# tskare/gpuaudiobench

Measured on AMD Instinct MI355X. Metric: audio_buffers_per_sec, higher is better.
Workload: dtype f32

## Files before the change

gpuaudiobench_amd/csrc/k_conv_accel.hip:

```cpp
#include <hip/hip_runtime.h>
#include <hip/hip_ext.h>

#include <cmath>
#include <cstdlib>
#include <algorithm>
#include <chrono>
#include <memory>
#include <mutex>
#include <string>
#include <thread>
#include <type_traits>
#include <utility>
#include <vector>

#include "gab_common.hpp"
#include "gab_fft.hpp"
#include "gab_plan.hpp"
#include "k_conv_fdl.hpp"

namespace gab {
namespace fft {

void build_twiddles(float* t) {
    for (int m = 0; m < kTwiddleN; ++m) {
// ... 380 lines not shown
    const float* __restrict__ hist, const float4* __restrict__ pmF, cf* __restrict__ carry,
    const cf* __restrict__ tw, int head) {
    __shared__ cf lds[2 * kLdsHalf];
    const int tid = threadIdx.x;
    const int q = blockIdx.x;
    const cf* const hp = reinterpret_cast<const cf*>(hist) + (size_t)q * kSlots * kB;
    cf* const cp = carry + (size_t)q * kCarrySlots * kB;
    using FB = fft::BlockFFT<kNB, 16, false>;
    using FBi = fft::BlockFFT<kNB, 16, true>;
    cf* const X = lds;
    cf* const Y = lds + kLdsHalf;
    cf zb[16];
    typename FB::Bases twb_base;
    FB::load_twiddles(twb_base, tw, tid);
#pragma unroll
    for (int r = 0; r < 16; ++r)
        zb[r] = hp[((head + 1 + (r >> 1)) & (kSlots - 1)) * kB + (r & 1) * kThreads + tid];
    float4 cb[16];
    load_spectra<kNB, 16>(cb, pmF + (size_t)q * kBinsB, tid);
    typename FB::Twiddles twb;
    FB::expand_twiddles(twb_base, twb);
    FB::run(zb, X, Y, twb, tid);
    cf zpb[16];
    partner_exchange<kNB, 16, true>(zb, zpb, X, tid);
    spectral_product<kNB, 16>(zb, zpb, cb, tid);
    FBi::template run<typename FB::Twiddles, 4>(zb, Y, X, twb, tid);
    cf* const c1 = cp + ((head + 1) & (kCarrySlots - 1)) * kB;
    cf* const c2 = cp + ((head + 2) & (kCarrySlots - 1)) * kB;
    c1[tid] = zb[12];
    c1[tid + kThreads] = zb[13];
    c2[tid] = zb[14];
    c2[tid + kThreads] = zb[15];
}

constexpr unsigned kRtSentinel = 0xffa5c3e1u;
__device__ __forceinline__ bool rt_pending(unsigned w) { return (w >> 24) == (kRtSentinel >> 24); }
constexpr size_t kRtUploadPiece = (size_t(4) << 20) - 256;
constexpr int kRtPollLimit = 1 << 21;
constexpr int kRtMaxGroups = 40;
constexpr size_t kBatchChunk = 256;
struct ConvRoundTrip {
    unsigned* stage;
    float* park;
    float* h_out;
    unsigned* counters;
    unsigned* done;
    const unsigned* landed;
    unsigned* error;
    unsigned epoch;
    int groups;
    unsigned bound[kRtMaxGroups + 1];
};

#ifdef GAB_ABLATE
__device__ unsigned long long g_rt_stamps[65 * 4];
#define GAB_RT_STAMP_MIN(g, i) do { if (threadIdx.x == 0) atomicMin(&g_rt_stamps[(g) * 4 + (i)], (unsigned long long)__builtin_amdgcn_s_memrealtime()); } while (0)
#define GAB_RT_STAMP_MAX(g, i) do { if (threadIdx.x == 0) atomicMax(&g_rt_stamps[(g) * 4 + (i)], (unsigned long long)__builtin_amdgcn_s_memrealtime()); } while (0)
#else
#define GAB_RT_STAMP_MIN(g, i) do {} while (0)
#define GAB_RT_STAMP_MAX(g, i) do {} while (0)
#endif

__device__ __forceinline__ unsigned rt_peek(const unsigned* p) {
    return __hip_atomic_load(p, __ATOMIC_RELAXED, __HIP_MEMORY_SCOPE_SYSTEM);
}
constexpr unsigned kRtErrWait = 1u, kRtErrTorn = 2u;

__global__ __launch_bounds__(kThreads) void conv_round_trip_check_kernel(unsigned* __restrict__ stage, const float* __restrict__ hist,
                                                                        unsigned* __restrict__ verdict, int slot) {
    const int tid = threadIdx.x, q = blockIdx.x;
    const cf* const hp = reinterpret_cast<const cf*>(hist) + ((size_t)q * kSlots + slot) * kB;
    unsigned* const row = stage + (size_t)(2 * q) * kB;
    const cf c0 = hp[tid], c1 = hp[tid + kThreads];
    const unsigned v0 = rt_peek(row + tid), v1 = rt_peek(row + tid + kThreads), v2 = rt_peek(row + kB + tid), v3 = rt_peek(row + kB + tid + kThreads);
    const bool torn = v0 != __float_as_uint(c0.x) || v2 != __float_as_uint(c0.y) || v1 != __float_as_uint(c1.x) || v3 != __float_as_uint(c1.y);
    if (torn) __hip_atomic_fetch_or(verdict, kRtErrTorn, __ATOMIC_RELAXED, __HIP_MEMORY_SCOPE_SYSTEM);
    __hip_atomic_store(row + tid, kRtSentinel, __ATOMIC_RELAXED, __HIP_MEMORY_SCOPE_SYSTEM);
    __hip_atomic_store(row + tid + kThreads, kRtSentinel, __ATOMIC_RELAXED, __HIP_MEMORY_SCOPE_SYSTEM);
    __hip_atomic_store(row + kB + tid, kRtSentinel, __ATOMIC_RELAXED, __HIP_MEMORY_SCOPE_SYSTEM);
    __hip_atomic_store(row + kB + tid + kThreads, kRtSentinel, __ATOMIC_RELAXED, __HIP_MEMORY_SCOPE_SYSTEM);
}

__global__ __launch_bounds__(kThreads, 2) void conv_round_trip_kernel(
    ConvRoundTrip rt, float* __restrict__ hist, const float4* __restrict__ pmA, const float4* __restrict__ pmB,
    const cf* __restrict__ tw, int T, int head) {
    __shared__ cf lds[2 * kLdsHalf];
    __shared__ int s_word;
    cf* const lds0 = lds;
    cf* const lds1 = lds + kLdsHalf;
    const int tid = threadIdx.x;
    const int q = blockIdx.x;
    const int ta = 2 * q;
    int g = 0;
    while (q >= (int)rt.bound[g + 1]) ++g;
    GAB_RT_STAMP_MIN(g, 0);
    cf* const hp = reinterpret_cast<cf*>(hist) + (size_t)q * kSlots * kB;
    using FA = fft::BlockFFT<kNA, 4, false>;
    using FAi = fft::BlockFFT<kNA, 4, true>;
    using FB = fft::BlockFFT<kNB, 16, false>;
    using FBi = fft::BlockFFT<kNB, 16, true>;

    cf zb[16];
    typename FB::Bases twb_base;
    FB::load_twiddles(twb_base, tw, tid);
#pragma unroll
    for (int r = 0; r < 16; ++r) zb[r] = hp[((head + (r >> 1)) & (kSlots - 1)) * kB + (r & 1) * kThreads + tid];
    const cf prev0 = zb[14], prev1 = zb[15];
    {
        float4 cb[16];
        load_spectra<kNB, 16>(cb, pmB + (size_t)q * kBinsB, tid);
        __builtin_amdgcn_sched_barrier(0);
        typename FB::Twiddles twb;
        FB::expand_twiddles(twb_base, twb);
        FB::run(zb, lds1, lds0, twb, tid);
        cf zpb[16];
        partner_exchange<kNB, 16, true>(zb, zpb, lds1, tid);
        spectral_product<kNB, 16>(zb, zpb, cb, tid);
        FBi::template run<typename FB::Twiddles, 2>(zb, lds0, lds1, twb, tid);
    }
    const cf far0 = zb[14], far1 = zb[15];

    float4 ca[4];
    load_spectra<kNA, 4>(ca, pmA + (size_t)q * kBinsA, tid);
    typename FA::Twiddles twa;
    {
        typename FA::Bases twa_base;
        FA::load_twiddles(twa_base, tw, tid);
        FA::expand_twiddles(twa_base, twa);
    }

    const unsigned* const row = rt.stage + (size_t)ta * kB;
    if (tid == 0) {
        int tries = 0, bad = 0;
        while (rt_pending(rt_peek(row + 2 * kB - 1))) {
            if ((++tries & 63) == 0 && rt_peek(rt.landed) == rt.epoch) break;
            if (tries > kRtPollLimit) { bad = 1; break; }
            __builtin_amdgcn_s_sleep(30);
        }
        s_word = bad;
    }
    __syncthreads();
    bool gave_up = s_word != 0;
    unsigned w[4];
    {
        int tries = 0;
        for (;;) {
            w[0] = rt_peek(row + tid);
            w[1] = rt_peek(row + tid + kThreads);
            w[2] = rt_peek(row + kB + tid);
            w[3] = rt_peek(row + kB + tid + kThreads);
            if (gave_up || !(rt_pending(w[0]) || rt_pending(w[1]) || rt_pending(w[2]) || rt_pending(w[3]))) break;
            if ((++tries & 15) == 0 && __hip_atomic_load(rt.landed, __ATOMIC_ACQUIRE, __HIP_MEMORY_SCOPE_SYSTEM) == rt.epoch) {
                w[0] = rt_peek(row + tid);
                w[1] = rt_peek(row + tid + kThreads);
                w[2] = rt_peek(row + kB + tid);
                w[3] = rt_peek(row + kB + tid + kThreads);
                break;
            }
            if (tries > kRtPollLimit) { gave_up = true; break; }
            __builtin_amdgcn_s_sleep(10);
        }
    }
    GAB_RT_STAMP_MAX(g, 1);
    if (gave_up) __hip_atomic_store(rt.error, kRtErrWait, __ATOMIC_RELAXED, __HIP_MEMORY_SCOPE_SYSTEM);

    cf za[4];
    za[0] = prev0;
    za[1] = prev1;
    za[2] = mk(__uint_as_float(w[0]), __uint_as_float(w[2]));
    za[3] = mk(__uint_as_float(w[1]), __uint_as_float(w[3]));
    hp[head * kB + tid] = za[2];
    hp[head * kB + kThreads + tid] = za[3];
    __syncthreads();
    FA::run(za, lds0, lds1, twa, tid);
    {
        cf zpa[4];
        partner_exchange<kNA, 4, true>(za, zpa, lds0, tid);
        spectral_product<kNA, 4>(za, zpa, ca, tid);
    }
    FAi::run(za, lds1, lds0, twa, tid);
    float ya0 = 0.f, yb0 = 0.f, ya1 = 0.f, yb1 = 0.f;
    ya0 += za[2].x; yb0 += za[2].y; ya1 += za[3].x; yb1 += za[3].y;
    ya0 += far0.x; yb0 += far0.y; ya1 += far1.x; yb1 += far1.y;

    {
        unsigned long long* const p0 = reinterpret_cast<unsigned long long*>(rt.park + (size_t)T * tid + ta);
        unsigned long long* const p1 = reinterpret_cast<unsigned long long*>(rt.park + (size_t)T * (tid + kThreads) + ta);
        const unsigned long long v0 = ((unsigned long long)__float_as_uint(yb0) << 32) | __float_as_uint(ya0);
        const unsigned long long v1 = ((unsigned long long)__float_as_uint(yb1) << 32) | __float_as_uint(ya1);
        __hip_atomic_store(p0, v0, __ATOMIC_RELAXED, __HIP_MEMORY_SCOPE_AGENT);
        __hip_atomic_store(p1, v1, __ATOMIC_RELAXED, __HIP_MEMORY_SCOPE_AGENT);
    }
    asm volatile("s_waitcnt vmcnt(0)" ::: "memory");
    __syncthreads();
    GAB_RT_STAMP_MAX(g, 2);
    const int first = rt.bound[g];
    const int members = (int)rt.bound[g + 1] - first;
    unsigned* const gw = rt.counters + 32 * g;
    if (tid == 0) {
        const unsigned old = __hip_atomic_fetch_add(&gw[0], 1u, __ATOMIC_RELAXED, __HIP_MEMORY_SCOPE_AGENT);
        int role = 1;
        if (old + 1u == rt.epoch * (unsigned)members) {
            role = 2;
            __hip_atomic_store(&gw[1], 0u, __ATOMIC_RELAXED, __HIP_MEMORY_SCOPE_AGENT);
            asm volatile("s_waitcnt vmcnt(0)" ::: "memory");
            __hip_atomic_store(&gw[2], rt.epoch, __ATOMIC_RELAXED, __HIP_MEMORY_SCOPE_AGENT);
        } else {
            int tries = 0;
            while (__hip_atomic_load(&gw[2], __ATOMIC_RELAXED, __HIP_MEMORY_SCOPE_AGENT) != rt.epoch) {
                if (++tries > (1 << 10)) { role = 0; break; }
                __builtin_amdgcn_s_sleep(3);
            }
        }
        s_word = role;
    }
    __syncthreads();
    const int role = s_word;
    if (role == 0) return;
    const int row_f4 = members / 2;
    const auto srd = __builtin_amdgcn_make_buffer_rsrc(rt.park, 0, (int)((size_t)T * kB * 4), 0x00020000);
    const int col0 = 2 * first;
    unsigned drained = 0;
    for (;;) {
        __syncthreads();
        if (tid == 0) s_word = (int)__hip_atomic_fetch_add(&gw[1], 1u, __ATOMIC_RELAXED, __HIP_MEMORY_SCOPE_AGENT);
        __syncthreads();
        const int share = s_word;
        if (share >= members) break;
        const int i = share * kThreads + tid;
        const int sidx = i / row_f4, c = i - sidx * row_f4;
        const auto raw = __builtin_amdgcn_raw_buffer_load_b128(srd, 4u * (unsigned)(T * sidx + col0 + 4 * c), 0, 16);
        typedef float f4v __attribute__((ext_vector_type(4)));
        const f4v val = {__uint_as_float(raw[0]), __uint_as_float(raw[1]), __uint_as_float(raw[2]), __uint_as_float(raw[3])};
        float* const dst = rt.h_out + (size_t)T * sidx + col0 + 4 * c;
        asm volatile("global_store_dwordx4 %0, %1, off sc0 sc1" ::"v"(dst), "v"(val) : "memory");
        ++drained;
        if (role != 2) break;
    }
    asm volatile("s_waitcnt vmcnt(0)" ::: "memory");
    __syncthreads();
    GAB_RT_STAMP_MAX(g, 3);
    if (tid == 0 && drained) {
        const unsigned old = __hip_atomic_fetch_add(&rt.counters[32 * rt.groups], drained, __ATOMIC_RELAXED, __HIP_MEMORY_SCOPE_AGENT);
        if (old + drained == rt.epoch * (unsigned)gridDim.x) {
            __hip_atomic_store(rt.done, rt.epoch, __ATOMIC_RELAXED, __HIP_MEMORY_SCOPE_SYSTEM);
            GAB_RT_STAMP_MAX(64, 0);
        }
    }
}

__global__ __launch_bounds__(kThreads, 2) void conv_batch_kernel(
    const float* __restrict__ in, float* __restrict__ out, float* __restrict__ hist,
    const float4* __restrict__ pmA, const float4* __restrict__ pmB,
    const cf* __restrict__ tw, int T, int head, int n_buffers) {
    __shared__ cf lds[2 * kLdsHalf];
    const size_t step = (size_t)T * kB;
    for (int nb = 0; nb < n_buffers; ++nb)
        conv_one_buffer<true, true, true>(in + nb * step, out + nb * step, hist, pmA, pmB, tw, T,
                                             (head + nb) & (kSlots - 1), lds);
}

constexpr int kBatchBarriers = 6;

struct ConvEngine {
    const unsigned* doorbell;
    unsigned* relay;
    unsigned* progress;
    unsigned* completed;
    unsigned* error;
    int ring;
    int poll_every_period;
    unsigned* started;
    unsigned* resident;
    unsigned long long idle_ticks;
};
constexpr double kEngineIdleSeconds = 4.0;

typedef unsigned u4 __attribute__((ext_vector_type(4)));

constexpr int kB12Threads = 768;
constexpr int kB12SpecCf = 4 * kBinsA * 2;
constexpr int kB12Tw1Cf = 16 * 15;
constexpr int kB12Lds = 6 * kWaveImg + 2 * kLdsHalf + kB12SpecCf + kB12Tw1Cf;

template <int N, int R, int R0, int R1, class PM>
__device__ __forceinline__ void load_spectra_part(float4 (&c)[R1 - R0], PM pm, int tid) {
    constexpr int NT = N / R;
#pragma unroll
    for (int r = R0; r < R1; ++r) {
        const int k = tid + r * NT;
        if (r < R / 2) c[r - R0] = pm[k];
        else if (r > R / 2) c[r - R0] = pm[N - k];
        else c[r - R0] = pm[tid == 0 ? k : N - k];
    }
}
template <int N, int R, int R0, int R1>
__device__ __forceinline__ void spectral_product_part(cf (&z)[R], const cf (&zraw)[R1 - R0], const float4 (&c)[R1 - R0], int tid) {
#pragma unroll
    for (int r = R0; r < R1; ++r) {
        cf P = mk(c[r - R0].x, c[r - R0].y), M = mk(c[r - R0].z, c[r - R0].w);
        if (r > R / 2 || (r == R / 2 && tid != 0)) z[r] = fft::cfma_cjcj(zraw[r - R0], M, fft::cmulc(z[r], P));
        else z[r] = fft::cfma_cj(zraw[r - R0], M, fft::cmul(z[r], P));
    }
}

#ifdef GAB_ABLATE
__device__ unsigned long long g_split_stamps[2 * 8 * 8192];
#define GAB_B12BAR(period, i)                                                                                         \
    do {                                                                                                              \
        if ((sp.debug & 64) && ((period) == 32 || (period) == 33) && lane == 0)                                       \
            g_split_stamps[(((size_t)blockIdx.x * 12 + w) * 2 + ((period) - 32)) * 6 + (i)] = __builtin_amdgcn_s_memrealtime(); \
        __syncthreads();                                                                                              \
    } while (0)
#else
#define GAB_B12BAR(period, i) __syncthreads()
#endif
__device__ __forceinline__ void conv_split_batch12_resident(
    const float* __restrict__ in, float* __restrict__ out, float* __restrict__ hist,
    const float4* __restrict__ pmA, const ConvSplit& sp, const cf* __restrict__ tw, int T, int head0, int n_buffers,
    cf* __restrict__ lds) {
    cf* const far_img = lds + 6 * kWaveImg;
    float4* const spec = reinterpret_cast<float4*>(far_img + 2 * kLdsHalf);
    cf* const tw1 = reinterpret_cast<cf*>(spec + 4 * kBinsA);
    const int tid = threadIdx.x;
    const int d = xcd_contiguous(blockIdx.x, gridDim.x);
    const size_t step = (size_t)T * kB;
    {
        const float4* const gA = pmA + (size_t)(2 * d) * kBinsA;
        const float4* const gA2 = sp.pmA2 + (size_t)(2 * d) * kBinsA;
        for (int i = tid; i < 2 * kBinsA; i += kB12Threads) { spec[i] = gA[i]; spec[2 * kBinsA + i] = gA2[i]; }
        if (tid < 16) {
            cf pw[15];
            fft::powers_of<16>(tw[tid * (fft::kTwiddleN / 256)], pw);
#pragma unroll
            for (int r = 0; r < 15; ++r) tw1[tid * 15 + r] = pw[r];
        }
    }
    __syncthreads();
    const int lane = tid & 63;
    const int w = __builtin_amdgcn_readfirstlane(tid >> 6);
    const unsigned rb = (unsigned)lane + ((unsigned)lane >> 4);
    auto in_slot = [&](int slot) -> const float* { return in + (size_t)slot * step; };
    auto idle_period = [&]() { for (int i = 0; i < kBatchBarriers; ++i) __syncthreads(); };

    if (w >= 4) {
        const int g = __builtin_amdgcn_readfirstlane((w - 4) >> 2);
        const int ft = (tid - kThreads) & (kThreads - 1);
        cf* const img = far_img + g * kLdsHalf;
        const int q = 2 * d + g;
        const cf* const hp = reinterpret_cast<const cf*>(hist) + (size_t)q * kSlots * kB;
        cf* const cg = sp.carry + (size_t)q * kCarrySlots * kB;
        const size_t ca = (size_t)(2 * q) * kB, cb_ = ca + kB;
        const float4* const pf = sp.pmF + (size_t)q * kBinsB;
        using B16 = fft::Butterfly<16, false>;
        using B16i = fft::Butterfly<16, true>;
        cf tw2[15];
        fft::powers_of<16>(tw[ft], tw2);
        auto opaque_t = [&]() -> unsigned { unsigned v = (unsigned)ft; asm volatile("" : "+v"(v)); return v; };
        auto w0_of = [](unsigned t) -> unsigned { return t * 17u; };
        auto rd_of = [](unsigned t) -> unsigned { return t + (t >> 4); };
        auto w1_of = [](unsigned t) -> unsigned { const unsigned b1 = (t >> 4) * 256u + (t & 15u); return b1 + (b1 >> 4); };
        auto tw1row_of = [&](unsigned t) -> const cf* { return tw1 + (t & 15u) * 15u; };
        auto load_window = [&](auto part_tag, int nb, cf (&z)[16]) {
            constexpr int PART = decltype(part_tag)::value;
            const int head = (head0 + nb) & (kSlots - 1);
            int fo = ft;
            asm volatile("" : "+v"(fo));
            if constexpr (PART == 0) {
                const float* const cur = in_slot(nb);
                z[14] = mk(cur[ca + fo], cur[cb_ + fo]);
                z[15] = mk(cur[ca + fo + kThreads], cur[cb_ + fo + kThreads]);
            }
            constexpr int BL0 = PART == 0 ? 4 : 0, BL1 = PART == 0 ? 7 : 4;
            if (nb >= kSlots - 1) {
#pragma unroll
                for (int bl = BL0; bl < BL1; ++bl) {
                    const float* const src = in_slot(nb - (7 - bl));
                    z[2 * bl] = mk(src[ca + fo], src[cb_ + fo]);
                    z[2 * bl + 1] = mk(src[ca + fo + kThreads], src[cb_ + fo + kThreads]);
                }
            } else {
#pragma unroll
                for (int bl = BL0; bl < BL1; ++bl) {
                    if (nb - 7 + bl >= 0) {
                        const float* const src = in_slot(nb - (7 - bl));
                        z[2 * bl] = mk(src[ca + fo], src[cb_ + fo]);
                        z[2 * bl + 1] = mk(src[ca + fo + kThreads], src[cb_ + fo + kThreads]);
                    } else {
                        const int s = ((head + 1 + bl) & (kSlots - 1)) * kB;
                        z[2 * bl] = hp[s + fo];
                        z[2 * bl + 1] = hp[s + kThreads + fo];
                    }
                }
            }
        };
        cf z[16], zn[16];
        auto first_half = [&](int nb) {
#pragma unroll
            for (int r = 0; r < 16; ++r) z[r] = zn[r];
            B16::run(z);
            {
                const unsigned w0 = w0_of(opaque_t());
#pragma unroll
                for (int r = 0; r < 16; ++r) img[w0 + r] = z[B16::out_slot(r)];
            }
            GAB_B12BAR(nb, 0);
            {
                const unsigned t = opaque_t(), rd = rd_of(t);
                const cf* const tw1row = tw1row_of(t);
#pragma unroll
                for (int r = 0; r < 16; ++r) z[r] = img[rd + 272 * r];
#pragma unroll
                for (int r = 1; r < 16; ++r) z[r] = fft::cmul(z[r], tw1row[r - 1]);
            }
            B16::run(z);
            GAB_B12BAR(nb, 1);
            {
                const unsigned w1 = w1_of(opaque_t());
#pragma unroll
                for (int r = 0; r < 16; ++r) img[w1 + 17 * r] = z[B16::out_slot(r)];
            }
            __builtin_amdgcn_sched_barrier(0);
            float4 clo[8], chi[8];
            {
                int fo = ft;
                asm volatile("" : "+v"(fo));
                load_spectra_part<kNB, 16, 0, 8>(clo, pf, fo);
            }
            __builtin_amdgcn_sched_barrier(0);
            GAB_B12BAR(nb, 2);
            {
                const unsigned rd = rd_of(opaque_t());
#pragma unroll
                for (int r = 0; r < 16; ++r) z[r] = img[rd + 272 * r];
            }
#pragma unroll
            for (int r = 1; r < 16; ++r) z[r] = fft::cmul(z[r], tw2[r - 1]);
            __builtin_amdgcn_sched_barrier(0);
            {
                int fo = ft;
                asm volatile("" : "+v"(fo));
                load_spectra_part<kNB, 16, 8, 16>(chi, pf, fo);
            }
            __builtin_amdgcn_sched_barrier(0);
            B16::run(z);
            GAB_B12BAR(nb, 3);
            {
                const unsigned t = opaque_t();
#pragma unroll
                for (int r = 0; r < 16; ++r) img[t + 256u * r] = z[B16::out_slot(r)];
            }
            GAB_B12BAR(nb, 4);
            {
                cf o[16];
#pragma unroll
                for (int r = 0; r < 16; ++r) o[r] = z[B16::out_slot(r)];
#pragma unroll
                for (int r = 0; r < 16; ++r) z[r] = o[r];
                const unsigned t = opaque_t();
                const cf* const pb = img + (kNB - 256 * 15) - t;
                cf zp[8];
                zp[0] = img[(kNB - t) & (kNB - 1)];
#pragma unroll
                for (int r = 1; r < 8; ++r) zp[r] = pb[256 * (15 - r)];
                spectral_product_part<kNB, 16, 0, 8>(z, zp, clo, ft);
#pragma unroll
                for (int r = 0; r < 8; ++r) zp[r] = pb[256 * (7 - r)];
                spectral_product_part<kNB, 16, 8, 16>(z, zp, chi, ft);
            }
            B16i::run(z);
            GAB_B12BAR(nb, 5);
        };
        auto second_half = [&](int period, int nb_done, int nb_next) {
            if (nb_next >= 0) {
                load_window(std::integral_constant<int, 0>{}, nb_next, zn);
            } else {
#pragma unroll
                for (int r = 0; r < 16; ++r) zn[r] = mk(0.0f, 0.0f);
            }
            GAB_B12BAR(period, 0);
            if (nb_done >= 0) {
                const unsigned w0 = w0_of(opaque_t());
#pragma unroll
                for (int r = 0; r < 16; ++r) img[w0 + r] = z[B16i::out_slot(r)];
            }
            GAB_B12BAR(period, 1);
            if (nb_done >= 0) {
                const unsigned t = opaque_t(), rd = rd_of(t);
                const cf* const tw1row = tw1row_of(t);
#pragma unroll
                for (int r = 0; r < 16; ++r) z[r] = img[rd + 272 * r];
#pragma unroll
                for (int r = 1; r < 16; ++r) z[r] = fft::cmulc(z[r], tw1row[r - 1]);
                B16i::run(z);
            }
            GAB_B12BAR(period, 2);
            if (nb_done >= 0) {
                const unsigned w1 = w1_of(opaque_t());
#pragma unroll
                for (int r = 0; r < 16; ++r) img[w1 + 17 * r] = z[B16i::out_slot(r)];
            }
            __builtin_amdgcn_sched_barrier(0);
            if (nb_next >= 0) load_window(std::integral_constant<int, 1>{}, nb_next, zn);
            __builtin_amdgcn_sched_barrier(0);
            GAB_B12BAR(period, 3);
            if (nb_done >= 0) {
                const unsigned rd = rd_of(opaque_t());
#pragma unroll
                for (int r = 0; r < 16; ++r) z[r] = img[rd + 272 * r];
#pragma unroll
                for (int r = 1; r < 16; ++r) z[r] = fft::cmulc(z[r], tw2[r - 1]);
                cf x12, x13, x14, x15;
                B16i::run_last4(z, x12, x13, x14, x15);
                const int head = (head0 + nb_done) & (kSlots - 1);
                cf* const c1 = cg + ((head + 1) & (kCarrySlots - 1)) * kB;
                cf* const c2 = cg + ((head + 2) & (kCarrySlots - 1)) * kB;
                c1[ft] = x12;
                c1[ft + kThreads] = x13;
                c2[ft] = x14;
                c2[ft + kThreads] = x15;
            }
            GAB_B12BAR(period, 4);
            if (nb_done >= 0) asm volatile("s_waitcnt vmcnt(0)" ::: "memory");
            GAB_B12BAR(period, 5);
        };
        const int first = (g - head0) & 1;
        int nb = 0;
        if (first == 1) {
            second_half(0, -1, 1 < n_buffers ? 1 : -1);
            nb = 1;
        } else if (n_buffers > 0) {
            load_window(std::integral_constant<int, 0>{}, 0, zn);
            load_window(std::integral_constant<int, 1>{}, 0, zn);
        }
        for (;;) {
            if (nb > n_buffers) break;
            if (nb < n_buffers) first_half(nb); else idle_period();
            ++nb;
            if (nb > n_buffers) break;
            second_half(nb, nb - 1 < n_buffers ? nb - 1 : -1, nb + 1 < n_buffers ? nb + 1 : -1);
            ++nb;
        }
    } else if (w < 2) {
        const int q = 2 * d + w;
        cf* const hp = reinterpret_cast<cf*>(hist) + (size_t)q * kSlots * kB;
        cf* const img = lds + w * kWaveImg;
        cf* const hand = lds + (2 + w) * kWaveImg;
        const float4* const sa = spec + w * kBinsA;
        const float4* const sa2 = spec + (2 + w) * kBinsA;
        using WF = fft::WaveFFT1024<false>;
        WF::Lean t;
        WF::load_twiddles(t, tw, lane);
        const size_t xoff = (size_t)(2 * q) * kB;
        cf z[16], prev[8], nxt[8];
        auto product_from_image = [&](cf (&v)[16], const float4* sp_lds) {
            {
                cf zp[8];
                float4 ch[8];
#pragma unroll
                for (int r = 0; r < 8; ++r) zp[r] = img[PadA16::at((kNA - (lane + 64 * r)) & (kNA - 1))];
                load_spectra_part<kNA, 16, 0, 8>(ch, sp_lds, lane);
                spectral_product_part<kNA, 16, 0, 8>(v, zp, ch, lane);
            }
            __builtin_amdgcn_sched_barrier(0);
            {
                cf zp[8];
                float4 ch[8];
#pragma unroll
                for (int r = 0; r < 8; ++r) zp[r] = img[PadA16::at((kNA - (lane + 64 * (8 + r))) & (kNA - 1))];
                load_spectra_part<kNA, 16, 8, 16>(ch, sp_lds, lane);
                spectral_product_part<kNA, 16, 8, 16>(v, zp, ch, lane);
            }
        };
        {
            const int s1 = ((head0 + kSlots - 1) & (kSlots - 1)) * kB, s2 = ((head0 + kSlots - 2) & (kSlots - 1)) * kB;
#pragma unroll
            for (int j = 0; j < 8; ++j) z[j] = hp[s2 + lane + 64 * j];
#pragma unroll
            for (int j = 0; j < 8; ++j) prev[j] = hp[s1 + lane + 64 * j];
            if (n_buffers > 0) {
                const float* const x0 = in_slot(0) + xoff;
#pragma unroll
                for (int j = 0; j < 8; ++j) nxt[j] = mk(x0[lane + 64 * j], x0[kB + lane + 64 * j]);
            }
#pragma unroll
            for (int j = 0; j < 8; ++j) z[8 + j] = prev[j];
            WF::run(z, img, t, lane, WF::NoHook());
#pragma unroll
            for (int r = 0; r < 16; ++r) img[rb + 68 * r] = z[r];
            __builtin_amdgcn_wave_barrier();
        }
        for (int nb = 0; nb < n_buffers; ++nb) {
            const int head = (head0 + nb) & (kSlots - 1);
            {
                cf share[16];
#pragma unroll
                for (int r = 0; r < 16; ++r) share[r] = img[rb + 68 * r];
                product_from_image(share, sa2);
                GAB_B12BAR(nb, 0);
#pragma unroll
                for (int r = 0; r < 16; ++r) hand[rb + 68 * r] = share[r];
            }
            __builtin_amdgcn_sched_barrier(0);
#pragma unroll
            for (int j = 0; j < 8; ++j) { z[j] = prev[j]; z[8 + j] = nxt[j]; }
            if (nb + kSlots >= n_buffers) {
#pragma unroll
                for (int j = 0; j < 8; ++j) hp[head * kB + lane + 64 * j] = nxt[j];
            }
#pragma unroll
            for (int j = 0; j < 8; ++j) prev[j] = nxt[j];
            if (nb + 1 < n_buffers) {
                int lo = lane;
                asm volatile("" : "+v"(lo));
                const float* const xa = in_slot(nb + 1) + xoff + lo;
#pragma unroll
                for (int j = 0; j < 8; ++j) nxt[j] = mk(xa[64 * j], xa[kB + 64 * j]);
            }
            WF::run(z, img, t, lane, [&](int i) { GAB_B12BAR(nb, 1 + i); });
            GAB_B12BAR(nb, 3);
#pragma unroll
            for (int r = 0; r < 16; ++r) img[rb + 68 * r] = z[r];
            __builtin_amdgcn_wave_barrier();
            product_from_image(z, sa);
            GAB_B12BAR(nb, 4);
#pragma unroll
            for (int r = 0; r < 16; ++r) hand[rb + 68 * r] = fft::cadd(z[r], hand[rb + 68 * r]);
            GAB_B12BAR(nb, 5);
        }
        idle_period();
    } else {
        const int pr = w - 2;
        const cf* const hand = lds + (2 + pr) * kWaveImg;
        cf* const img = lds + (4 + pr) * kWaveImg;
        const cf* const other = lds + (4 + (1 - pr)) * kWaveImg;
        const cf* const cg = sp.carry + (size_t)(2 * d + pr) * kCarrySlots * kB;
        using WFi = fft::WaveFFT1024<true>;
        WFi::Lean t;
        WFi::load_twiddles(t, tw, lane);
        idle_period();
        for (int nb = 1; nb <= n_buffers; ++nb) {
            const int b = nb - 1;
            const int head = (head0 + b) & (kSlots - 1);
            float* const outb = out + (size_t)b * step;
            cf z[16], y[8], park[8];
#pragma unroll
            for (int r = 0; r < 16; ++r) z[r] = hand[rb + 68 * r];
            {
                int lo = lane;
                asm volatile("" : "+v"(lo));
                const unsigned long long* const cy = reinterpret_cast<const unsigned long long*>(cg + (head & (kCarrySlots - 1)) * kB + lo);
#pragma unroll
                for (int j = 0; j < 8; ++j) {
                    const unsigned long long v = __hip_atomic_load(cy + 64 * j, __ATOMIC_RELAXED, __HIP_MEMORY_SCOPE_AGENT);
                    park[j] = mk(__uint_as_float((unsigned)v), __uint_as_float((unsigned)(v >> 32)));
                }
            }
            GAB_B12BAR(nb, 0);
            WFi::run(z, img, t, lane, [&](int i) { GAB_B12BAR(nb, 1 + i); });
#pragma unroll
            for (int j = 0; j < 8; ++j) y[j] = fft::cadd(z[8 + j], park[j]);
            GAB_B12BAR(nb, 3);
            if (pr == 0) {
#pragma unroll
                for (int j = 0; j < 4; ++j) img[lane + 64 * j] = y[4 + j];
            } else {
#pragma unroll
                for (int j = 0; j < 4; ++j) img[lane + 64 * j] = y[j];
            }
            GAB_B12BAR(nb, 4);
            {
                float* const o0 = outb + 4 * (size_t)d;
                if (pr == 0) {
#pragma unroll
                    for (int j = 0; j < 4; ++j) {
                        const cf theirs = other[lane + 64 * j];
                        *reinterpret_cast<float4*>(o0 + (size_t)T * (lane + 64 * j)) = make_float4(y[j].x, y[j].y, theirs.x, theirs.y);
                    }
                } else {
#pragma unroll
                    for (int j = 0; j < 4; ++j) {
                        const cf theirs = other[lane + 64 * j];
                        *reinterpret_cast<float4*>(o0 + (size_t)T * (lane + 64 * (4 + j))) = make_float4(theirs.x, theirs.y, y[4 + j].x, y[4 + j].y);
                    }
                }
            }
            GAB_B12BAR(nb, 5);
        }
    }
}

__global__ __launch_bounds__(kB12Threads) void conv_split_batch12_kernel(
    const float* __restrict__ in, float* __restrict__ out, float* __restrict__ hist,
    const float4* __restrict__ pmA, ConvSplit sp, const cf* __restrict__ tw, int T, int head0, int n_buffers) {
    __shared__ __attribute__((aligned(16))) cf lds[kB12Lds];
    conv_split_batch12_resident(in, out, hist, pmA, sp, tw, T, head0, n_buffers, lds);
}

#ifdef GAB_ABLATE
#define GAB_E12BAR(i)                                                                                                 \
    do {                                                                                                              \
        if ((sp.debug & 64) && (nb == 4000 || nb == 4001) && lane == 0)                                               \
            g_split_stamps[(((size_t)blockIdx.x * 12 + w) * 2 + (nb - 4000)) * 6 + (i)] = __builtin_amdgcn_s_memrealtime(); \
        __syncthreads();                                                                                              \
    } while (0)
#else
#define GAB_E12BAR(i) __syncthreads()
#endif
__device__ __forceinline__ void conv_split_engine12_resident(
    const float* __restrict__ in, float* __restrict__ out, float* __restrict__ hist,
    const float4* __restrict__ pmA, const ConvSplit& sp, const cf* __restrict__ tw, int T, int head0,
    const ConvEngine& eng, cf* __restrict__ lds, unsigned* __restrict__ s_door) {
    constexpr bool ENGINE = true;
    constexpr int n_buffers = 0;
    (void)ENGINE; (void)n_buffers;
    cf* const far_img = lds + 6 * kWaveImg;
    float4* const spec = reinterpret_cast<float4*>(far_img + 2 * kLdsHalf);
    cf* const tw1 = reinterpret_cast<cf*>(spec + 4 * kBinsA);
    const int tid = threadIdx.x;
    const int d = xcd_contiguous(blockIdx.x, gridDim.x);
    const size_t step = (size_t)T * kB;
    {
        const float4* const gA = pmA + (size_t)(2 * d) * kBinsA;
        const float4* const gA2 = sp.pmA2 + (size_t)(2 * d) * kBinsA;
        for (int i = tid; i < 2 * kBinsA; i += kB12Threads) { spec[i] = gA[i]; spec[2 * kBinsA + i] = gA2[i]; }
        if (tid < 16) {
            cf pw[15];
            fft::powers_of<16>(tw[tid * (fft::kTwiddleN / 256)], pw);
#pragma unroll
            for (int r = 0; r < 15; ++r) tw1[tid * 15 + r] = pw[r];
        }
    }
    constexpr int kPoller = 2 * 64;
    auto read_door = [&]() -> unsigned {
        if (blockIdx.x == 0) {
            const unsigned v = __hip_atomic_load(eng.doorbell, __ATOMIC_RELAXED, __HIP_MEMORY_SCOPE_SYSTEM);
            __hip_atomic_store(eng.relay, v, __ATOMIC_RELAXED, __HIP_MEMORY_SCOPE_AGENT);
            return v;
        }
        return __hip_atomic_load(eng.relay, __ATOMIC_RELAXED, __HIP_MEMORY_SCOPE_AGENT);
    };
    if (tid == 0) {
        s_door[2] = 0;
        const unsigned before = __hip_atomic_fetch_add(eng.started, 1u, __ATOMIC_RELAXED, __HIP_MEMORY_SCOPE_AGENT);
        if (before == 0) __hip_atomic_store(&eng.resident[0], 1u, __ATOMIC_RELAXED, __HIP_MEMORY_SCOPE_SYSTEM);
        if (before + 1 == gridDim.x) __hip_atomic_store(&eng.resident[1], gridDim.x, __ATOMIC_RELAXED, __HIP_MEMORY_SCOPE_SYSTEM);
    }
    __syncthreads();
    const int lane = tid & 63;
    const int w = __builtin_amdgcn_readfirstlane(tid >> 6);
    const unsigned rb = (unsigned)lane + ((unsigned)lane >> 4);
    const bool aggregator = blockIdx.x == (gridDim.x > 1 ? 1u : 0u);
    unsigned reported = 0;
    auto aggregate_request = [&](u4& a, u4& b) {
        const auto srd = __builtin_amdgcn_make_buffer_rsrc(eng.progress, 0, (int)(8u * gridDim.x), 0x00020000);
        a = __builtin_amdgcn_raw_buffer_load_b128(srd, 32u * (unsigned)lane, 0, 16);
        b = __builtin_amdgcn_raw_buffer_load_b128(srd, 32u * (unsigned)lane + 16u, 0, 16);
    };
    auto aggregate_report = [&](const u4& a, const u4& b) {
        const unsigned words = 2u * gridDim.x;
        auto pick = [&](unsigned v, unsigned idx) { return idx < words ? v : 0xffffffffu; };
        unsigned m = min(min(min(pick(a[0], 8u * lane), pick(a[1], 8u * lane + 1)), min(pick(a[2], 8u * lane + 2), pick(a[3], 8u * lane + 3))),
                         min(min(pick(b[0], 8u * lane + 4), pick(b[1], 8u * lane + 5)), min(pick(b[2], 8u * lane + 6), pick(b[3], 8u * lane + 7))));
#pragma unroll
        for (int o = 32; o > 0; o >>= 1) m = min(m, (unsigned)__shfl_xor((int)m, o));
        if (m != reported) {
            reported = m;
            if (lane == 0) __hip_atomic_store(eng.completed, m, __ATOMIC_RELAXED, __HIP_MEMORY_SCOPE_SYSTEM);
        }
    };
    auto gate = [&](int nb, bool idle) -> int {
        {
            if (idle && __builtin_amdgcn_readfirstlane(s_door[2]) != 0) return -1;
            bool look = !idle;
            for (;;) {
                if (look) {
                    const unsigned D = __builtin_amdgcn_readfirstlane(s_door[nb & 1]);
                    const int pub = (int)(D & 0x3fffffffu);
                    const bool stop = (D >> 31) != 0, flush = ((D >> 30) & 1u) != 0;
                    if (pub >= nb + 2 || ((stop || flush) && pub >= nb + 1)) return pub;
                    if (stop) return -1;
                }
                look = true;
                __syncthreads();
                if (w == 2) {
                    unsigned v = 0;
                    int tries = 0;
                    const unsigned long long t_poll = __builtin_amdgcn_s_memrealtime();
                    for (;;) {
                        u4 pa, pb;
                        if (aggregator) aggregate_request(pa, pb);
                        unsigned mine = 0;
                        if (lane == 0) mine = read_door();
                        v = __builtin_amdgcn_readfirstlane(mine);
                        if (aggregator) aggregate_report(pa, pb);
                        const int p2 = (int)(v & 0x3fffffffu);
                        if (p2 >= nb + 2 || (v >> 31) || (((v >> 30) & 1u) && p2 >= nb + 1)) break;
                        if ((++tries & 255) == 0 && __builtin_amdgcn_s_memrealtime() - t_poll > eng.idle_ticks) {
                            if (lane == 0) {
                                __hip_atomic_store(eng.error, 1u, __ATOMIC_RELAXED, __HIP_MEMORY_SCOPE_SYSTEM);
                                s_door[2] = 1;
                            }
                            v = 0x80000000u | (unsigned)(p2 < nb ? p2 : nb);
                            break;
                        }
                        __builtin_amdgcn_s_sleep(6);
                    }
                    if (lane == 0) s_door[nb & 1] = v;
                }
                __syncthreads();
            }
        }
    };
    auto in_slot = [&](int slot) -> const float* { return in + (size_t)slot * step; };
    auto next_slot = [&](int slot) -> int { return (ENGINE && slot + 1 == eng.ring) ? 0 : slot + 1; };
    auto ld = [](const float* p) -> float {
        if constexpr (ENGINE)
            return __hip_atomic_load(p, __ATOMIC_RELAXED, __HIP_MEMORY_SCOPE_SYSTEM);
        else return *p;
    };

    auto idle_period = [&]() { for (int i = 0; i < kBatchBarriers; ++i) __syncthreads(); };

    if (w >= 4) {
        const int g = __builtin_amdgcn_readfirstlane((w - 4) >> 2);
        const int ft = (tid - kThreads) & (kThreads - 1);
        cf* const img = far_img + g * kLdsHalf;
        const int q = 2 * d + g;
        const cf* const hp = reinterpret_cast<const cf*>(hist) + (size_t)q * kSlots * kB;
        cf* const cg = sp.carry + (size_t)q * kCarrySlots * kB;
        const size_t ca = (size_t)(2 * q) * kB, cb_ = ca + kB;
        const float4* const pf = sp.pmF + (size_t)q * kBinsB;
        using B16 = fft::Butterfly<16, false>;
        using B16i = fft::Butterfly<16, true>;
        const cf tw2_base = tw[ft];
        auto tw2_of = [&](cf (&w)[15]) {
            cf b = tw2_base;
            asm volatile("" : "+v"(b.x), "+v"(b.y));
            fft::powers_of<16>(b, w);
        };
        auto opaque_t = [&]() -> unsigned { unsigned v = (unsigned)ft; asm volatile("" : "+v"(v)); return v; };
        auto w0_of = [](unsigned t) -> unsigned { return t * 17u; };
        auto rd_of = [](unsigned t) -> unsigned { return t + (t >> 4); };
        auto w1_of = [](unsigned t) -> unsigned { const unsigned b1 = (t >> 4) * 256u + (t & 15u); return b1 + (b1 >> 4); };
        auto tw1row_of = [&](unsigned t) -> const cf* { return tw1 + (t & 15u) * 15u; };
        auto load_window = [&](auto part_tag, auto first_tag, int nb, int slot, int slot_before, cf (&z)[16]) {
            constexpr int PART = decltype(part_tag)::value;
            constexpr bool FIRST = decltype(first_tag)::value;
            const int head = (head0 + nb) & (kSlots - 1);
            int fo = ft;
            asm volatile("" : "+v"(fo));
            if constexpr (PART == 0) {
                const float* const cur = in_slot(slot);
                z[14] = mk(ld(cur + ca + fo), ld(cur + cb_ + fo));
                z[15] = mk(ld(cur + ca + fo + kThreads), ld(cur + cb_ + fo + kThreads));
                if constexpr (!FIRST) {
                    const float* const prv = in_slot(slot_before);
                    z[12] = mk(ld(prv + ca + fo), ld(prv + cb_ + fo));
                    z[13] = mk(ld(prv + ca + fo + kThreads), ld(prv + cb_ + fo + kThreads));
                } else {
                    const int s6 = ((head + kSlots - 1) & (kSlots - 1)) * kB;
                    z[12] = hp[s6 + fo];
                    z[13] = hp[s6 + kThreads + fo];
                }
#pragma unroll
                for (int bl = 4; bl < 6; ++bl) {
                    const int sb = ((head + 1 + bl) & (kSlots - 1)) * kB;
                    z[2 * bl] = hp[sb + fo];
                    z[2 * bl + 1] = hp[sb + kThreads + fo];
                }
            } else {
#pragma unroll
                for (int bl = 0; bl < 4; ++bl) {
                    const int sb = ((head + 1 + bl) & (kSlots - 1)) * kB;
                    z[2 * bl] = hp[sb + fo];
                    z[2 * bl + 1] = hp[sb + kThreads + fo];
                }
            }
        };
        cf z[16], zn[16];
        auto first_half = [&](int nb) {
#pragma unroll
            for (int r = 0; r < 16; ++r) z[r] = zn[r];
            B16::run(z);
            {
                const unsigned w0 = w0_of(opaque_t());
#pragma unroll
                for (int r = 0; r < 16; ++r) img[w0 + r] = z[B16::out_slot(r)];
            }
            GAB_E12BAR(0);
            {
                const unsigned t = opaque_t(), rd = rd_of(t);
                const cf* const tw1row = tw1row_of(t);
#pragma unroll
                for (int r = 0; r < 16; ++r) z[r] = img[rd + 272 * r];
#pragma unroll
                for (int r = 1; r < 16; ++r) z[r] = fft::cmul(z[r], tw1row[r - 1]);
            }
            B16::run(z);
            GAB_E12BAR(1);
            {
                const unsigned w1 = w1_of(opaque_t());
#pragma unroll
                for (int r = 0; r < 16; ++r) img[w1 + 17 * r] = z[B16::out_slot(r)];
            }
            __builtin_amdgcn_sched_barrier(0);
            float4 clo[8], chi[8];
            {
                int fo = ft;
                asm volatile("" : "+v"(fo));
                load_spectra_part<kNB, 16, 0, 8>(clo, pf, fo);
            }
            __builtin_amdgcn_sched_barrier(0);
            GAB_E12BAR(2);
            {
                const unsigned rd = rd_of(opaque_t());
#pragma unroll
                for (int r = 0; r < 16; ++r) z[r] = img[rd + 272 * r];
            }
            {
                cf tw2[15];
                tw2_of(tw2);
#pragma unroll
                for (int r = 1; r < 16; ++r) z[r] = fft::cmul(z[r], tw2[r - 1]);
            }
            __builtin_amdgcn_sched_barrier(0);
            {
                int fo = ft;
                asm volatile("" : "+v"(fo));
                load_spectra_part<kNB, 16, 8, 16>(chi, pf, fo);
            }
            __builtin_amdgcn_sched_barrier(0);
            B16::run(z);
            GAB_E12BAR(3);
            {
                const unsigned t = opaque_t();
#pragma unroll
                for (int r = 0; r < 16; ++r) img[t + 256u * r] = z[B16::out_slot(r)];
            }
            GAB_E12BAR(4);
            {
                cf o[16];
#pragma unroll
                for (int r = 0; r < 16; ++r) o[r] = z[B16::out_slot(r)];
#pragma unroll
                for (int r = 0; r < 16; ++r) z[r] = o[r];
                const unsigned t = opaque_t();
                const cf* const pb = img + (kNB - 256 * 15) - t;
                cf zp[8];
                zp[0] = img[(kNB - t) & (kNB - 1)];
#pragma unroll
                for (int r = 1; r < 8; ++r) zp[r] = pb[256 * (15 - r)];
                spectral_product_part<kNB, 16, 0, 8>(z, zp, clo, ft);
#pragma unroll
                for (int r = 0; r < 8; ++r) zp[r] = pb[256 * (7 - r)];
                spectral_product_part<kNB, 16, 8, 16>(z, zp, chi, ft);
            }
            B16i::run(z);
            GAB_E12BAR(5);
        };
        auto second_half = [&](int period, int nb_done, int nb_next, int slot_next, int slot_now) {
            const int nb = period;
            (void)nb;
            if (nb_next >= 0) {
                load_window(std::integral_constant<int, 0>{}, std::false_type{}, nb_next, slot_next, slot_now, zn);
            } else {
#pragma unroll
                for (int r = 0; r < 16; ++r) zn[r] = mk(0.0f, 0.0f);
            }
            GAB_E12BAR(0);
            if (nb_done >= 0) {
                const unsigned w0 = w0_of(opaque_t());
#pragma unroll
                for (int r = 0; r < 16; ++r) img[w0 + r] = z[B16i::out_slot(r)];
            }
            GAB_E12BAR(1);
            if (nb_done >= 0) {
                const unsigned t = opaque_t(), rd = rd_of(t);
                const cf* const tw1row = tw1row_of(t);
#pragma unroll
                for (int r = 0; r < 16; ++r) z[r] = img[rd + 272 * r];
#pragma unroll
                for (int r = 1; r < 16; ++r) z[r] = fft::cmulc(z[r], tw1row[r - 1]);
                B16i::run(z);
            }
            GAB_E12BAR(2);
            if (nb_done >= 0) {
                const unsigned w1 = w1_of(opaque_t());
#pragma unroll
// ... 1597 lines not shown
```

Measured before the change: 202,000.

## Split near-partition spectral products between forward and inverse FFT waves

The near-partition spectral product and accumulation, previously done entirely by the forward-FFT waves, is now split in half. Forward waves compute bins 0-7 and the inverse waves compute bins 8-15 from the shared LDS image, so the work is spread across more waves in the batched-12 split convolution kernel. This adds a prologue with block-wide syncs and restructures the handoff buffers. It aims to shorten the critical path of the forward waves, at the cost of extra barriers and more work and register pressure on the inverse waves.

Measured after the change: 206,700, median of 6. 1.02x the previous value.

```diff
diff --git a/gpuaudiobench_amd/csrc/k_conv_accel.hip b/gpuaudiobench_amd/csrc/k_conv_accel.hip
--- a/gpuaudiobench_amd/csrc/k_conv_accel.hip
+++ b/gpuaudiobench_amd/csrc/k_conv_accel.hip
@@ -706,6 +706,15 @@
         if (r > R / 2 || (r == R / 2 && tid != 0)) z[r] = fft::cfma_cjcj(zraw[r - R0], M, fft::cmulc(z[r], P));
         else z[r] = fft::cfma_cj(zraw[r - R0], M, fft::cmul(z[r], P));
     }
+}
+template <int R0, int R1>
+__device__ __forceinline__ void near_product_half(cf (&v)[16], const cf* fimg, const float4* sp_lds, int lane) {
+    cf zp[R1 - R0];
+    float4 ch[R1 - R0];
+#pragma unroll
+    for (int r = R0; r < R1; ++r) zp[r - R0] = fimg[PadA16::at((kNA - (lane + 64 * r)) & (kNA - 1))];
+    load_spectra_part<kNA, 16, R0, R1>(ch, sp_lds, lane);
+    spectral_product_part<kNA, 16, R0, R1>(v, zp, ch, lane);
 }
 
 #ifdef GAB_ABLATE
@@ -930,12 +939,14 @@
         };
         const int first = (g - head0) & 1;
         int nb = 0;
+        if (first == 0 && n_buffers > 0) {
+            load_window(std::integral_constant<int, 0>{}, 0, zn);
+            load_window(std::integral_constant<int, 1>{}, 0, zn);
+        }
+        __syncthreads();
         if (first == 1) {
             second_half(0, -1, 1 < n_buffers ? 1 : -1);
             nb = 1;
-        } else if (n_buffers > 0) {
-            load_window(std::integral_constant<int, 0>{}, 0, zn);
-            load_window(std::integral_constant<int, 1>{}, 0, zn);
         }
         for (;;) {
             if (nb > n_buffers) break;
@@ -957,25 +968,6 @@
         WF::load_twiddles(t, tw, lane);
         const size_t xoff = (size_t)(2 * q) * kB;
         cf z[16], prev[8], nxt[8];
-        auto product_from_image = [&](cf (&v)[16], const float4* sp_lds) {
-            {
-                cf zp[8];
-                float4 ch[8];
-#pragma unroll
-                for (int r = 0; r < 8; ++r) zp[r] = img[PadA16::at((kNA - (lane + 64 * r)) & (kNA - 1))];
-                load_spectra_part<kNA, 16, 0, 8>(ch, sp_lds, lane);
-                spectral_product_part<kNA, 16, 0, 8>(v, zp, ch, lane);
-            }
-            __builtin_amdgcn_sched_barrier(0);
-            {
-                cf zp[8];
-                float4 ch[8];
-#pragma unroll
-                for (int r = 0; r < 8; ++r) zp[r] = img[PadA16::at((kNA - (lane + 64 * (8 + r))) & (kNA - 1))];
-                load_spectra_part<kNA, 16, 8, 16>(ch, sp_lds, lane);
-                spectral_product_part<kNA, 16, 8, 16>(v, zp, ch, lane);
-            }
-        };
         {
             const int s1 = ((head0 + kSlots - 1) & (kSlots - 1)) * kB, s2 = ((head0 + kSlots - 2) & (kSlots - 1)) * kB;
 #pragma unroll
@@ -992,19 +984,15 @@
             WF::run(z, img, t, lane, WF::NoHook());
 #pragma unroll
             for (int r = 0; r < 16; ++r) img[rb + 68 * r] = z[r];
-            __builtin_amdgcn_wave_barrier();
+            __syncthreads();
         }
         for (int nb = 0; nb < n_buffers; ++nb) {
             const int head = (head0 + nb) & (kSlots - 1);
-            {
-                cf share[16];
-#pragma unroll
-                for (int r = 0; r < 16; ++r) share[r] = img[rb + 68 * r];
-                product_from_image(share, sa2);
-                GAB_B12BAR(nb, 0);
-#pragma unroll
-                for (int r = 0; r < 16; ++r) hand[rb + 68 * r] = share[r];
-            }
+            cf share[16];
+#pragma unroll
+            for (int r = 0; r < 8; ++r) share[r] = img[rb + 68 * r];
+            near_product_half<0, 8>(share, img, sa2, lane);
+            GAB_B12BAR(nb, 0);
             __builtin_amdgcn_sched_barrier(0);
 #pragma unroll
             for (int j = 0; j < 8; ++j) { z[j] = prev[j]; z[8 + j] = nxt[j]; }
@@ -1022,34 +1010,67 @@
                 for (int j = 0; j < 8; ++j) nxt[j] = mk(xa[64 * j], xa[kB + 64 * j]);
             }
             WF::run(z, img, t, lane, [&](int i) { GAB_B12BAR(nb, 1 + i); });
+#pragma unroll
+            for (int r = 0; r < 16; ++r) img[rb + 68 * r] = z[r];
             GAB_B12BAR(nb, 3);
-#pragma unroll
-            for (int r = 0; r < 16; ++r) img[rb + 68 * r] = z[r];
-            __builtin_amdgcn_wave_barrier();
-            product_from_image(z, sa);
+            near_product_half<0, 8>(z, img, sa, lane);
             GAB_B12BAR(nb, 4);
 #pragma unroll
-            for (int r = 0; r < 16; ++r) hand[rb + 68 * r] = fft::cadd(z[r], hand[rb + 68 * r]);
+            for (int r = 0; r < 8; ++r) hand[rb + 68 * r] = fft::cadd(z[r], share[r]);
             GAB_B12BAR(nb, 5);
         }
         idle_period();
     } else {
         const int pr = w - 2;
-        const cf* const hand = lds + (2 + pr) * kWaveImg;
+        cf* const hand = lds + (2 + pr) * kWaveImg;
+        const cf* const fimg = lds + pr * kWaveImg;
+        const float4* const sa = spec + pr * kBinsA;
+        const float4* const sa2 = spec + (2 + pr) * kBinsA;
         cf* const img = lds + (4 + pr) * kWaveImg;
         const cf* const other = lds + (4 + (1 - pr)) * kWaveImg;
         const cf* const cg = sp.carry + (size_t)(2 * d + pr) * kCarrySlots * kB;
         using WFi = fft::WaveFFT1024<true>;
         WFi::Lean t;
         WFi::load_twiddles(t, tw, lane);
-        idle_period();
+        cf ws[16], sum[8];
+        auto product_half = [&](const float4* sp_lds) {
+#pragma unroll
+            for (int r = 8; r < 16; ++r) ws[r] = fimg[rb + 68 * r];
+            near_product_half<8, 16>(ws, fimg, sp_lds, lane);
+        };
+        auto store_share = [&]() {
+#pragma unroll
+            for (int r = 8; r < 16; ++r) hand[rb + 68 * r] = ws[r];
+        };
+        auto sum_halves = [&]() {
+#pragma unroll
+            for (int j = 0; j < 8; ++j) sum[j] = fft::cadd(ws[8 + j], hand[rb + 68 * (8 + j)]);
+        };
+        __syncthreads();
+        if (n_buffers > 0) {
+            product_half(sa2);
+            GAB_B12BAR(0, 0);
+            store_share();
+            GAB_B12BAR(0, 1);
+            GAB_B12BAR(0, 2);
+            GAB_B12BAR(0, 3);
+            product_half(sa);
+            GAB_B12BAR(0, 4);
+            sum_halves();
+            GAB_B12BAR(0, 5);
+        } else {
+            idle_period();
+        }
         for (int nb = 1; nb <= n_buffers; ++nb) {
+            const bool products = nb < n_buffers;
             const int b = nb - 1;
             const int head = (head0 + b) & (kSlots - 1);
             float* const outb = out + (size_t)b * step;
             cf z[16], y[8], park[8];
 #pragma unroll
-            for (int r = 0; r < 16; ++r) z[r] = hand[rb + 68 * r];
+            for (int r = 0; r < 8; ++r) z[r] = hand[rb + 68 * r];
+#pragma unroll
+            for (int j = 0; j < 8; ++j) z[8 + j] = sum[j];
             {
                 int lo = lane;
                 asm volatile("" : "+v"(lo));
@@ -1060,7 +1081,11 @@
                     park[j] = mk(__uint_as_float((unsigned)v), __uint_as_float((unsigned)(v >> 32)));
                 }
             }
+            __builtin_amdgcn_sched_barrier(0);
+            if (products) product_half(sa2);
             GAB_B12BAR(nb, 0);
+            if (products) store_share();
+            __builtin_amdgcn_sched_barrier(0);
             WFi::run(z, img, t, lane, [&](int i) { GAB_B12BAR(nb, 1 + i); });
 #pragma unroll
             for (int j = 0; j < 8; ++j) y[j] = fft::cadd(z[8 + j], park[j]);
@@ -1072,6 +1097,8 @@
 #pragma unroll
                 for (int j = 0; j < 4; ++j) img[lane + 64 * j] = y[j];
             }
+            __builtin_amdgcn_sched_barrier(0);
+            if (products) product_half(sa);
             GAB_B12BAR(nb, 4);
             {
                 float* const o0 = outb + 4 * (size_t)d;
@@ -1089,6 +1116,7 @@
                     }
                 }
             }
+            if (products) sum_halves();
             GAB_B12BAR(nb, 5);
         }
     }
```
